# ChuhanZhou/News_Recommendation_Model

Measured on AMD Instinct MI355X. Metric: train impressions/sec, higher is better.
Workload: dtype f32

## Files before the change

### include/nrm_hotpath.h

```cpp
#ifndef NRM_HOTPATH_H
#define NRM_HOTPATH_H

#ifdef __cplusplus
extern "C" {
#endif

#define NRM_ABI_VERSION 7
#define NRM_OK 0
#define NRM_EINVAL (-1)
#define NRM_ELAUNCH (-2)

typedef void* nrm_stream_t;

int nrm_abi_version(void);
const char* nrm_last_error(void);
int nrm_build_flags(void);
const char* nrm_source_digest(void);
const char* nrm_build_info(void);


#define NRM_MMA_F32 0
#define NRM_MMA_BF16 1
#define NRM_MMA_BF16X3 2
long nrm_pwattn_packed_floats(int D);
int nrm_pwattn_pack_wp(const float* fc1_weight, int ld, int D, int mma, float* packed, nrm_stream_t stream);
int nrm_pwattn_fwd(const float* t, const float* h, const float* u, const float* v, const float* packed_wp,
                   const float* w2, const float* b2, float* z, float* s,
                   int B, int T, int H, int D, int mma, nrm_stream_t stream);

#define NRM_DZ_F32 0
#define NRM_DZ_HL4 1
int nrm_pwattn_bwd_dz(float* z_inout, const float* ds, const float* w2, float* dw2, float* db2, float* du, float* dv,
                      int B, int T, int H, int D, int dz_format, nrm_stream_t stream);
int nrm_pwattn_bwd_nsplit(int B, int T, int H, int D, int mma);
int nrm_pwattn_bwd_contract(const float* dz, const float* t, const float* h, const float* wp, int ldwp,
                            float* dt, float* dh, float* ws,
                            int B, int T, int H, int D, int passes, int mma, int dz_format, nrm_stream_t stream);
int nrm_pwattn_bwd_form(int T, int H, int D, int pass, int mma, int dz_format);
int nrm_pwattn_bwd_rw_supported(int D, int mma);
long nrm_pwattn_bwd_rw_packed_floats(int D, int mma);
int nrm_pwattn_bwd_rw_pack(const float* fc1_weight, int ld, int D, int mma, float* packed, nrm_stream_t stream);
int nrm_pwattn_bwd_rw_dtdh(const float* dz_hl4, const float* t, const float* h, const float* packed, float* dt, float* dh,
                           int B, int T, int H, int D, int mma, nrm_stream_t stream);

int nrm_pwattn_bwd_dp_supported(int D, int H);
long nrm_pwattn_bwd_dp_packed_floats(int D, int H);
int nrm_pwattn_bwd_dp_pack(const float* fc1_weight, int ld, int D, int H, float* packed, nrm_stream_t stream);
int nrm_pwattn_bwd_dp_dtdh(const float* dz, const float* t, const float* h, const float* packed, float* dt, float* dh,
                           int B, int T, int H, int D, nrm_stream_t stream);

#define NRM_EPI_BIAS 0
#define NRM_EPI_GELU 1
#define NRM_EPI_DGELU 2
#define NRM_EPI_MUL 3
long nrm_gemm_packed_floats(int nrows, int ncols, int mma);
int nrm_gemm_nt_bf16_supported(int M, int K, int mma);
int nrm_gemm_pack(const float* src, long row_stride, long col_stride, int nrows, int ncols, float* packed,
                  nrm_stream_t stream);
typedef struct {
    const float* src; const float* src2; float sign2;
    long row_stride, col_stride; int nrows, ncols;
    float* packed;
    int mma;
} nrm_pack_desc;
int nrm_gemm_pack_multi(const nrm_pack_desc* descs, int n, nrm_stream_t stream);
int nrm_gemm_nt(const float* x, int ldx, int M, const float* packed, int N, int K, const float* bias,
                float* y, int ldy, float* z, int ldz, const float* m, int ldm, int epilogue, int mma, nrm_stream_t stream);
int nrm_gemm_tn_nsplit(int ncols_i, int ncols_j, int R, int mma);
int nrm_gemm_tn(const float* A, int lda, int ncols_i, const float* B, int ldb, int ncols_j, int R,
                float* ws, int ldws, float* colsum, float* zero_out, long zero_n, int mma, nrm_stream_t stream);

int nrm_slab_reduce(const float* ws, int nsplit, int nj, int ldws, int ni, float* out, long out_istride, long out_jstride,
                    float* out2, long out2_istride, long out2_jstride, float sign2,
                    const float* vec, float* vec_out, nrm_stream_t stream);
typedef struct nrm_slab_desc {
    const float* ws; int nsplit, nj, ldws, ni;
    float* out; long out_istride, out_jstride;
    float* out2; long out2_istride, out2_jstride; float sign2;
    const float* vec; float* vec_out;
} nrm_slab_desc;
int nrm_slab_reduce_multi(const nrm_slab_desc* descs, int n, nrm_stream_t stream);

int nrm_head_fold(const float* w_o1, const float* b_o1, const float* w_m2, const float* b_m2, int P, int Q, int R,
                  float* packed_fwd, float* packed_bwd, float* bias, nrm_stream_t stream);
int nrm_head_fold_bwd(const float* dwp, int ldp, const float* dbp, const float* w_o1, const float* w_m2, const float* b_m2,
                      int P, int Q, int R, float* dw_o1, float* dw_m2, float* db_o1, float* db_m2, nrm_stream_t stream);

int nrm_colreduce(int mode, const float* x, const float* dy, const float* mean, const float* rstd,
                  float* s0, float* s1, int R, int N, int ld, nrm_stream_t stream);
int nrm_bn_finalize(int stage, const float* s, float* out, float* running, int R, int N, float momentum, float eps,
                    nrm_stream_t stream);
// ... 98 lines not shown
```

### news_recommendation_model_amd/csrc/capi.hip

```cpp
#include <stdarg.h>
#include <stdint.h>
#include <stdio.h>
#include <stdlib.h>
#include <vector>

#include "../../include/nrm_hotpath.h"
#include "pwattn.hpp"
#include "gemm.hpp"
#include "head.hpp"
#include "pool_loss.hpp"
#include "frontend.hpp"
#include "scoring.hpp"
#include "compact.hpp"

static thread_local char g_err[512] = "";

static int fail(int code, const char* fmt, ...) {
    va_list ap;
    va_start(ap, fmt);
    vsnprintf(g_err, sizeof(g_err), fmt, ap);
    va_end(ap);
    return code;
}
static int check_hip(hipError_t e, const char* what) {
// ... 201 lines not shown
    if (!fc1_weight || !packed) return fail(NRM_EINVAL, "nrm_pwattn_bwd_dp_pack: null pointer");
    if (D <= 0 || D % 4 || ld < 4 * D) return fail(NRM_EINVAL, "nrm_pwattn_bwd_dp_pack: D=%d ld=%d (need D%%4==0, ld>=4D)", D, ld);
    if (!nrm_pwattn_bwd_dp_supported(D, H)) return fail(NRM_EINVAL, "nrm_pwattn_bwd_dp_pack: D=%d H=%d has no dP-walk backward", D, H);
    return check_hip(nrm::pwattn_bwd_dp_pack_launch(fc1_weight + 3 * (long)D, ld, D, H, packed, (hipStream_t)stream), "bwd_dp_pack");
}

int nrm_pwattn_bwd_dp_dtdh(const float* dz, const float* t, const float* h, const float* packed, float* dt, float* dh,
                           int B, int T, int H, int D, nrm_stream_t stream) {
    if (int rc = check_dims("nrm_pwattn_bwd_dp_dtdh", B, T, H, D)) return rc;
    if (!dz || !t || !h || !packed || !dt || !dh) return fail(NRM_EINVAL, "nrm_pwattn_bwd_dp_dtdh: null pointer");
    if (!nrm_pwattn_bwd_dp_supported(D, H)) return fail(NRM_EINVAL, "nrm_pwattn_bwd_dp_dtdh: D=%d H=%d has no dP-walk backward (D %% 4 == 0, H >= 16)", D, H);
    if ((long)(63 / H + 2) * T * H * D * 4 >= (1L << 31)) return fail(NRM_EINVAL, "nrm_pwattn_bwd_dp_dtdh: the dz blocks of one row block exceed 2^31 bytes");
    if ((long)B * H * D * 4 >= (1L << 31) || (long)B * T * D * 4 >= (1L << 31)) return fail(NRM_EINVAL, "nrm_pwattn_bwd_dp_dtdh: t or h exceeds 2^31 bytes");
    if (B == 0) return NRM_OK;
    nrm::BwdDpParams p = {};
    p.dz = dz; p.t = t; p.h = h; p.wimg = packed; p.dt = dt; p.dh = dh; p.B = B; p.T = T; p.H = H; p.D = D;
    p.w_bytes = (unsigned)(nrm_pwattn_bwd_dp_packed_floats(D, H) * 4);
    p.t_bytes = (unsigned)((long)B * T * D * 4); p.h_bytes = (unsigned)((long)B * H * D * 4);
    return check_hip(nrm::pwattn_bwd_dp_launch(p, (hipStream_t)stream), "bwd_dp_dtdh");
}

int nrm_pwattn_bwd_nsplit(int B, int T, int H, int D, int mma) {
    if (B <= 0 || T <= 0 || H <= 0 || D <= 0) return 0;
    return bwd_bt_plan(B, T, D, mma).nsplit;
}

int nrm_pwattn_bwd_contract(const float* dz, const float* t, const float* h, const float* wp, int ldwp,
                            float* dt, float* dh, float* ws, int B, int T, int H, int D, int passes, int mma,
                            int dz_format, nrm_stream_t stream) {
    if (int rc = check_dims("nrm_pwattn_bwd_contract", B, T, H, D)) return rc;
    if (int rc = check_mma("nrm_pwattn_bwd_contract", mma)) return rc;
    if (passes != 1 && passes != 2 && passes != 3 && passes != 4) return fail(NRM_EINVAL, "nrm_pwattn_bwd_contract: passes=%d", passes);
    if (!bwd_dz_format_ok(passes, mma, dz_format))
        return fail(NRM_EINVAL, "nrm_pwattn_bwd_contract: passes=%d mma=%d with dz_format=%d (only the dW_p-only pass, 4, of the bf16 arithmetics reads NRM_DZ_HL4)", passes, mma, dz_format);
    if (!dz || !t || !h || !wp) return fail(NRM_EINVAL, "nrm_pwattn_bwd_contract: null pointer");
    if (((passes & 1) && (!dt || !ws)) || ((passes & 2) && !dh) || (passes == 4 && !ws)) return fail(NRM_EINVAL, "nrm_pwattn_bwd_contract: null output");
    if (ldwp < D || ldwp % 4) return fail(NRM_EINVAL, "nrm_pwattn_bwd_contract: ldwp=%d", ldwp);
    if (B == 0) return NRM_OK;
    for (int pass : {passes == 4 ? 4 : passes & 1, passes & 2}) {
        if (!pass) continue;
        const BwdPass a = bwd_pass(pass, dz, t, h, wp, ldwp, dt, dh, ws, B, T, H, D, mma, dz_format);
        if (int rc = check_hip(nrm::bwd_e_launch(a.p, a.pl, a.with_dw, mma, (hipStream_t)stream), pass == 2 ? "bwd_e pass 2" : "bwd_e pass 1")) return rc;
    }
    return NRM_OK;
}

int nrm_pwattn_bwd_form(int T, int H, int D, int pass, int mma, int dz_format) {
    if (check_dims("nrm_pwattn_bwd_form", 1, T, H, D) || check_mma("nrm_pwattn_bwd_form", mma)) return -1;
    if ((pass != 1 && pass != 2 && pass != 4) || !bwd_dz_format_ok(pass, mma, dz_format)) return -1;
    const BwdPass a = bwd_pass(pass, nullptr, nullptr, nullptr, nullptr, D, nullptr, nullptr, nullptr, 1, T, H, D, mma, dz_format);
    const nrm::BwdEForm f = nrm::bwd_e_select(a.p, a.pl, a.with_dw, mma, nrm::bwd_e_knobs());
    if (f.family == nrm::BWD_E_REFUSED) return -1;
    return f.family | (f.exact ? 4 : 0) | (a.pl.DT == 5 ? 8 : 0) | (f.with_dw ? 16 : 0) | (f.with_dt ? 32 : 0) | (f.xhl4 ? 64 : 0);
}

static bool al16(const void* p) { return ((uintptr_t)p & 15) == 0; }

long nrm_gemm_packed_floats(int nrows, int ncols, int mma) {
    if (nrows <= 0 || ncols <= 0) return 0;
    if (mma == NRM_MMA_BF16 || mma == NRM_MMA_BF16X3)
        return (long)((nrows + 15) / 16) * ((ncols + 31) / 32) * (mma == NRM_MMA_BF16X3 ? 2 : 1) * 256 + 1024;
    const nrm::GemmNtPlan pl = nrm::gemm_nt_plan(nrows);
    return (long)((ncols + 15) / 16) * pl.rows * 16 + 1024;
}

int nrm_gemm_nt_bf16_supported(int M, int K, int mma) { return nrm::gemm_nt_rx_bm(M, K, mma) ? 1 : 0; }

int nrm_gemm_pack(const float* src, long row_stride, long col_stride, int nrows, int ncols, float* packed,
                  nrm_stream_t stream) {
    if (!src || !packed || nrows <= 0 || ncols <= 0) return fail(NRM_EINVAL, "nrm_gemm_pack: bad argument");
    const nrm::GemmNtPlan pl = nrm::gemm_nt_plan(nrows);
    return check_hip(nrm::pack_rows_launch(src, row_stride, col_stride, nrows, ncols, pl.rows, (ncols + 15) / 16, packed,
                                           (hipStream_t)stream), "pack_rows");
}

int nrm_gemm_pack_multi(const nrm_pack_desc* descs, int n, nrm_stream_t stream) {
    if (n < 0 || (n > 0 && !descs)) return fail(NRM_EINVAL, "nrm_gemm_pack_multi: bad argument");
    for (int lo = 0; lo < n; lo += nrm::PACK_MAX) {
        const int m = n - lo < nrm::PACK_MAX ? n - lo : nrm::PACK_MAX;
        nrm::PackTable tab = {};
        long mx = 0;
        for (int i = 0; i < m; ++i) {
            const nrm_pack_desc& d = descs[lo + i];
            if (!d.src || !d.packed || d.nrows <= 0 || d.ncols <= 0) return fail(NRM_EINVAL, "nrm_gemm_pack_multi: entry %d is malformed", lo + i);
            const nrm::GemmNtPlan pl = nrm::gemm_nt_plan(d.nrows);
            nrm::PackEntry& e = tab.e[i];
            e.src = d.src; e.src2 = d.src2; e.dst = d.packed; e.rs = d.row_stride; e.cs = d.col_stride;
            e.nrows = d.nrows; e.ncols = d.ncols; e.rows = pl.rows; e.kchunks = (d.ncols + 15) / 16; e.sign2 = d.sign2; e.fmt = 0;
            if (d.mma == NRM_MMA_BF16 || d.mma == NRM_MMA_BF16X3) {
                e.fmt = d.mma == NRM_MMA_BF16X3 ? 2 : 1; e.rows = (d.nrows + 15) / 16 * 16; e.kchunks = (d.ncols + 31) / 32;
            } else if (d.mma != NRM_MMA_F32) return fail(NRM_EINVAL, "nrm_gemm_pack_multi: entry %d: mma=%d", lo + i, d.mma);
            const long total = e.fmt ? (long)(e.rows / 16) * e.kchunks * 512 : (long)e.kchunks * e.rows * 16;
            if (total > mx) mx = total;
        }
        if (int rc = check_hip(nrm::pack_rows_multi_launch(tab, m, mx, (hipStream_t)stream), "pack_rows_multi")) return rc;
    }
    return NRM_OK;
}

int nrm_gemm_nt(const float* x, int ldx, int M, const float* packed, int N, int K, const float* bias,
                float* y, int ldy, float* z, int ldz, const float* m, int ldm, int epilogue, int mma, nrm_stream_t stream) {
    if (!x || !packed || !y) return fail(NRM_EINVAL, "nrm_gemm_nt: null pointer");
    if (M < 0 || N <= 0 || K <= 0) return fail(NRM_EINVAL, "nrm_gemm_nt: M=%d N=%d K=%d", M, N, K);
    if (ldx % 4 || ldy % 4 || ldx < K || ldy < N || !al16(x) || !al16(y))
        return fail(NRM_EINVAL, "nrm_gemm_nt: ldx=%d ldy=%d must be multiples of 4 covering K=%d / N=%d, rows 16-B aligned", ldx, ldy, K, N);
    if (epilogue != NRM_EPI_BIAS && (!z || ldz % 4 || ldz < N || !al16(z)))
// ... 501 lines not shown
```

### news_recommendation_model_amd/csrc/pwattn.hpp

```cpp
#pragma once
#include <hip/hip_runtime.h>

namespace nrm {

struct FwdParams {
    const float* t;
    const float* h;
    const float* u;
    const float* v;
    const float* wp;
    const float* w2;
    const float* b2;
    float* z;
    float* s;
    long M;
    int T, H, D;
    int ldt, ldh, ldu, ldv;
    unsigned wp_bytes, t_bytes, h_bytes;
    int rows;
    int kchunks;
    int nchunks;
};
struct RaggedTabs {
    const int* cand_imp;
    const int* cand_off;
    int B, N;
    int max_count;
    const int* hist_off;
    const int* tile_pre;
    const int4* tile_tab;
    int R, Mt, k_max;
};
struct FwdPlan { int NT, MT, nchunks, rows, kchunks; };
FwdPlan pwattn_fwd_plan(int D);
hipError_t pwattn_fwd_launch(const FwdParams& p, const FwdPlan& pl, int mma, hipStream_t st);
hipError_t pwattn_fwd_ragged_launch(const FwdParams& p, const FwdPlan& pl, const RaggedTabs& rg, hipStream_t st);
hipError_t pwattn_fwd_hragged_launch(const FwdParams& p, const FwdPlan& pl, const RaggedTabs& rg, hipStream_t st);
hipError_t pack_wp_launch(const float* w, int ldw, int D, const FwdPlan& pl, int mma, float* packed, hipStream_t st);
struct RwPlan { int nts, nsplit, rows, k32, wimg; };
RwPlan pwattn_rw_plan(int D, int mma);
bool pwattn_fwd_uses_rw(int D, int mma);
hipError_t pwattn_fwd_rw_launch(const FwdParams& p, int mma, hipStream_t st);
hipError_t pwattn_fwd_rw_ragged_launch(const FwdParams& p, const RaggedTabs& rg, hipStream_t st);
hipError_t pwattn_fwd_rw_hragged_launch(const FwdParams& p, const RaggedTabs& rg, hipStream_t st);
hipError_t pack_wp_bf16_launch(const float* w, int ldw, int D, int mma, float* packed, hipStream_t st);

struct BwdEParams {
    const float* X; long xs1, xs2, xrs;
    const float* Y; long ys1, yrs;
    const float* wp; int ldwp;
    const float* srow; int lds_;
    float* out; int ldo;
    float* ws;
    int G, G2, R, D;
    int gps;
    int nkw, ndcol;
    int nsplit;
    int interleave;
    int x_hl4;
    int with_dt;
    int order;
};
struct BwdEPlan { int DT, KT, ndcol, nkw, nsplit, gps; };
BwdEPlan bwd_e_plan(int D, int G, int target_waves, int min_gps = 1, int mma = 0);
enum BwdEFamily { BWD_E_REFUSED = -1, BWD_E_SERIAL = 0, BWD_E_PIPE = 1, BWD_DW_DIRECT = 2, BWD_DW_R32 = 3 };
struct BwdEKnobs { bool pipe, dw_direct, dw_r32; };
BwdEKnobs bwd_e_knobs();
struct BwdEForm {
    int family;
    bool with_dw, with_dt, xhl4; int ks;
    bool exact; int mma;
};
BwdEForm bwd_e_select(const BwdEParams& p, const BwdEPlan& pl, bool with_dw, int mma, const BwdEKnobs& knobs);
hipError_t bwd_e_launch(const BwdEParams& p, const BwdEPlan& pl, bool with_dw, int mma, hipStream_t st);
hipError_t bwd_dz_launch(float* z, const float* ds, const float* w2, float* dw2, float* db2, float* du, float* dv,
                         int B, int T, int H, int D, int dz_format, hipStream_t st);

struct BwdRwParams {
    const float* dz;
    const float* t;
    const float* h;
    const float* wimg;
    float* dt;
    float* dh;
    int B, T, H, D;
    unsigned w_bytes;
    int tsplit;
};
struct BwdRwPlan { int ng, kc, nks, wimg, k32, rows; };
BwdRwPlan pwattn_bwd_rw_plan(int D, int mma);
long pwattn_bwd_rw_packed_floats(int D, int mma);
hipError_t pwattn_bwd_rw_pack_launch(const float* wp, int ldw, int D, int mma, float* packed, hipStream_t st);
hipError_t pwattn_bwd_rw_launch(const BwdRwParams& p, int mma, hipStream_t st);

struct BwdDpParams {
    const float* dz;
    const float* t;
    const float* h;
    const float* wimg;
    float* dt;
    float* dh;
    int B, T, H, D;
    unsigned w_bytes, t_bytes, h_bytes;
    int rows, kchunks, nchunks;
    long steps;
};
struct BwdDpPlan { int NT, nchunks, rows, kchunks; };
BwdDpPlan pwattn_bwd_dp_plan(int D, int H);
long pwattn_bwd_dp_packed_floats(int D, int H);
hipError_t pwattn_bwd_dp_pack_launch(const float* wp, int ldw, int D, int H, float* packed, hipStream_t st);
hipError_t pwattn_bwd_dp_launch(BwdDpParams p, hipStream_t st);

int pwattn_fwd_diag_flags();
int pwattn_fwd_rw_diag_flags();
int pwattn_bwd_rw_diag_flags();
int pwattn_bwd_dp_diag_flags();
int pwattn_bwd_diag_flags();

}
```

### news_recommendation_model_amd/csrc/pwattn_bwd.hip

```cpp
#include <cstdlib>
#include <type_traits>
#ifndef NRM_PRIO
#define NRM_PRIO 0
#endif
#ifndef NRM_PIPE_SGB
#define NRM_PIPE_SGB 1
#endif
#ifndef NRM_EPI_AHEAD
#define NRM_EPI_AHEAD 1
#endif
#ifndef NRM_DIAG_GELU_AT_LOAD
#define NRM_DIAG_GELU_AT_LOAD 0
#endif
#ifndef NRM_DIAG_NOEPI
#define NRM_DIAG_NOEPI 0
#endif
#ifndef NRM_DIAG_NOATOM
#define NRM_DIAG_NOATOM 0
#endif
#ifndef NRM_DIAG_NOLOAD
#define NRM_DIAG_NOLOAD 0
#endif
#include "common.hpp"
#include "pwattn.hpp"
// ... 675 lines not shown
            if (lg >= g_hi) return;
            if (ls == 0) open_group(lg);
            const u32x4 va = __builtin_amdgcn_raw_buffer_load_b128(rx, vx4, ls * xstep, 0);
            const u32x4 vb = __builtin_amdgcn_raw_buffer_load_b128(ry, vy4, ls * ystep, 0);
#pragma unroll
            for (int e = 0; e < 4; ++e) { a[e] = __uint_as_float(va[e]); b[e] = __uint_as_float(vb[e]); }
            if (KT > 4) a[4] = __uint_as_float(__builtin_amdgcn_raw_buffer_load_b32(rx, vx1, ls * xstep, 0));
            if (DT > 4) b[4] = __uint_as_float(__builtin_amdgcn_raw_buffer_load_b32(ry, vy1, ls * ystep, 0));
            if (++ls == nsteps) { ls = 0; lg += g_step; }
        };
        int cs = 0;
        auto consume = [&](const float (&a)[KT], const float (&b)[DT]) {
            if (cs == 0) {
#pragma unroll
                for (int jt = 0; jt < DT; ++jt) sr_cur[jt] = sr_nxt[jt];
            }
            float bs[DT];
#pragma unroll
            for (int jt = 0; jt < DT; ++jt) bs[jt] = b[jt] * sr_cur[jt];
            e_mfma<KT, DT>(dW, a, bs);
            if (++cs == nsteps) cs = 0;
        };
        const int ngroups = (g_hi - g_lo + g_step - 1) / g_step;
        const int total = ngroups * nsteps;
#pragma unroll
        for (int u = 0; u < NSET; ++u) request(a[u], b[u]);
        for (int n = 0; n < total; n += NSET) {
#pragma unroll
            for (int u = 0; u < NSET; ++u)
                if (u == 0 || n + u < total) {
                    consume(a[u], b[u]);
                    request(a[u], b[u]);
                }
        }
    }

    float* wsp = p.ws + (long)split * D * D;
#pragma unroll
    for (int jt = 0; jt < DT; ++jt) {
        const int d = d0 + tn_col<DT>(jt, r16);
        if (!(EXACT || d < D)) continue;
        float* row = wsp + (long)d * D + k0;
#pragma unroll
        for (int e = 0; e < 4; ++e) {
            const int kk = 16 * q + 4 * e;
            if (EXACT || k0 + kk < D)
                *reinterpret_cast<f32x4*>(row + kk) = f32x4{dW[0][jt][e], dW[1][jt][e], dW[2][jt][e], dW[3][jt][e]};
        }
        if (KT > 4 && (EXACT || k0 + 64 + 4 * q < D)) *reinterpret_cast<f32x4*>(row + 64 + 4 * q) = dW[KT - 1][jt];
    }
#endif
}

template <int KT, int DT, bool EXACT>
__global__ __launch_bounds__(256, 2) void bwd_e_pipe_kernel(const BwdEParams p) {
#if defined(__HIP_DEVICE_COMPILE__)
    constexpr int PE = (DT + 1) & ~1;
    constexpr int LDK = KT * 16 + 8;
    __shared__ __attribute__((aligned(16))) float smem[DT * 16 * LDK + 4 * DT * 16];
    float* wpt = smem;
    const int tid = threadIdx.x;
    const int lane = tid & 63;
    const int wave = __builtin_amdgcn_readfirstlane(tid >> 6);
    float* bounce = smem + DT * 16 * LDK + wave * (DT * 16);
    const int r16 = lane & 15, q = lane >> 4;
    const int D = p.D, R = p.R;

    const ETile tl = e_tile<KT, DT, false>(p);
    const int d0 = tl.d0, k0 = tl.k0, sgrp = tl.sgrp;

    for (int idx = tid; idx < KT * 16 * DT * 4; idx += 256) {
        const int kl = idx / (DT * 4), d4 = idx - kl * (DT * 4);
        const int k = k0 + kl, d = d0 + 4 * d4;
        f32x4 w = f32x4{0.f, 0.f, 0.f, 0.f};
        if (k < D && d < D) w = *reinterpret_cast<const f32x4*>(p.wp + (long)k * p.ldwp + d);
#pragma unroll
        for (int e = 0; e < 4; ++e) wpt[tile_pos(4 * d4 + e) * LDK + tile_pos(kl)] = w[e];
    }
    __syncthreads();

    const int split = sgrp * 4 + wave;
    if (split >= p.nsplit) return;
    const EGroups gr = e_groups<false>(p, sgrp, wave);
    const int g_lo = gr.lo, g_hi = gr.hi;
    if (g_lo >= g_hi) return;
    const int nsteps = (R + 3) >> 2;

    const unsigned vx4 = (EXACT || k0 + 4 * r16 < D) ? (unsigned)((long)q * p.xrs + k0 + 4 * r16) * 4u : BUF_OOB;
    const unsigned vx1 = (EXACT || k0 + 64 + r16 < D) ? (unsigned)((long)q * p.xrs + k0 + 64 + r16) * 4u : BUF_OOB;
    const unsigned vy4 = (EXACT || d0 + 4 * r16 < D) ? (unsigned)((long)q * p.yrs + d0 + 4 * r16) * 4u : BUF_OOB;
    const unsigned vy1 = (EXACT || d0 + 64 + r16 < D) ? (unsigned)((long)q * p.yrs + d0 + 64 + r16) * 4u : BUF_OOB;
    const unsigned xbytes = (unsigned)(((long)(R - 1) * p.xrs + D) * 4);
    const unsigned ybytes = (unsigned)(((long)(R - 1) * p.yrs + D) * 4);
    const int xstep = (int)(p.xrs * 16), ystep = (int)(p.yrs * 16);

    float a0[KT], b0[DT], a1[KT], b1[DT];
    __amdgpu_buffer_rsrc_t rx, ry, rxn, ryn;
    auto open_group = [&](int gg, __amdgpu_buffer_rsrc_t& ox, __amdgpu_buffer_rsrc_t& oy) {
        const EOperands o = e_open(p, gg, xbytes, ybytes);
        ox = o.x; oy = o.y;
    };
    bool diag_first = true;
    auto load_step = [&](__amdgpu_buffer_rsrc_t dx, __amdgpu_buffer_rsrc_t dy, float (&a)[KT], float (&b)[DT], int s) {
        if (NRM_DIAG_NOLOAD == 1 && !(diag_first && s < 2)) return;
        const u32x4 va = __builtin_amdgcn_raw_buffer_load_b128(dx, vx4, s * xstep, 0);
        const u32x4 vb = __builtin_amdgcn_raw_buffer_load_b128(dy, vy4, s * ystep, 0);
// ... 173 lines not shown
                f32x4 c = f32x4{0.f, 0.f, 0.f, 0.f};
                if (MMA == 2) {
                    c = __builtin_amdgcn_mfma_f32_16x16x32_bf16(al, ybf[jt], c, 0, 0, 0);
                    c = __builtin_amdgcn_mfma_f32_16x16x32_bf16(af, ybl[jt], c, 0, 0, 0);
                }
                E[it][jt] = __builtin_amdgcn_mfma_f32_16x16x32_bf16(af, ybf[jt], c, 0, 0, 0);
            }
        }
#pragma unroll
        for (int jt = 0; jt < DT; ++jt)
#pragma unroll
            for (int it = 0; it < KT; ++it) dW[it][jt] += E[it][jt] * sr[jt];
    }

    float* wsp = p.ws + (long)split * D * D;
#pragma unroll
    for (int jt = 0; jt < DT; ++jt) {
        const int d = d0 + 4 * r16 + jt;
        if (!(EXACT || d < D)) continue;
        float* row = wsp + (long)d * D + k0;
#pragma unroll
        for (int e = 0; e < 4; ++e) {
            const int kk = 16 * q + 4 * e;
            if (EXACT || k0 + kk < D)
                *reinterpret_cast<f32x4*>(row + kk) = f32x4{dW[0][jt][e], dW[1][jt][e], dW[2][jt][e], dW[3][jt][e]};
        }
    }
#endif
}

BwdEPlan bwd_e_plan(int D, int G, int target_waves, int min_gps, int mma) {
    const int n16 = (D + 15) / 16;
    const int c5 = (n16 + 4) / 5 * 5, c4 = (n16 + 3) / 4 * 4;
    BwdEPlan pl;
    if (c5 < c4) { pl.DT = 5; pl.KT = 5; } else { pl.DT = 4; pl.KT = 4; }
    if (mma != 0) { pl.DT = 4; pl.KT = 4; }
    pl.ndcol = (n16 + pl.DT - 1) / pl.DT;
    pl.nkw = (n16 + pl.KT - 1) / pl.KT;
    const int tiles = pl.ndcol * pl.nkw;
    int ns = target_waves / tiles / 4 * 4;
    if (min_gps > 1 && ns > G / min_gps) {
        const int one_round = 2048 / tiles / 4 * 4;
        if (one_round >= 4 && one_round < ns) ns = one_round;
    }
    if (ns < 4) ns = 4;
    if (ns > G) ns = G > 0 ? G : 1;
    pl.gps = (G + ns - 1) / ns;
    pl.nsplit = pl.gps > 0 ? (G + pl.gps - 1) / pl.gps : 1;
    return pl;
}

BwdEKnobs bwd_e_knobs() {
    auto on = [](const char* name) { const char* e = getenv(name); return !(e && e[0] == '0'); };
    return {on("NRM_BH_PIPE"), on("NRM_DW_DIRECT"), on("NRM_DW_R32")};
}

BwdEForm bwd_e_select(const BwdEParams& p, const BwdEPlan& pl, bool with_dw, int mma, const BwdEKnobs& knobs) {
    const int KT = pl.KT, DT = pl.DT;
    const BwdEForm refused = {BWD_E_REFUSED, false, false, false, 0, false, mma};
    BwdEForm f = {BWD_E_SERIAL, with_dw, true, false, DT, p.D % (16 * KT) == 0 && p.D % (16 * DT) == 0, mma};
    if (KT != 4) {
        if (mma != 0) return refused;
    } else if (mma == 1 || mma == 2) {
        if (!p.with_dt && !p.x_hl4) {
            if (!with_dw) return refused;
            f.with_dt = false;
        } else if (!p.with_dt || p.x_hl4) {
            if (!with_dw || p.with_dt || !p.x_hl4) return refused;
            f.with_dt = false; f.xhl4 = true;
            if (knobs.dw_r32 && p.R <= 32) f.family = BWD_DW_R32;
        }
        return f;
    }
    f.mma = 0;
    if (with_dw && !p.with_dt) {
        if (p.x_hl4) return refused;
        f.with_dt = false;
        if (knobs.dw_direct && (p.R + 3) / 4 >= DW_SETS) f.family = BWD_DW_DIRECT;
    } else if (!with_dw && knobs.pipe && (p.R + 3) / 4 >= ((DT + 1) & ~1) + 2) {
        f.family = BWD_E_PIPE;
    }
    return f;
}

template <class F>
static void with_tile_exact_mma(int tile, bool exact, int mma, F&& f) {
    auto go = [&](auto t, auto m) { return exact ? f(t, std::true_type{}, m) : f(t, std::false_type{}, m); };
    using T4 = std::integral_constant<int, 4>;
    if (tile == 5) return go(std::integral_constant<int, 5>{}, std::integral_constant<int, 0>{});
    if (mma == 1) return go(T4{}, std::integral_constant<int, 1>{});
    if (mma == 2) return go(T4{}, std::integral_constant<int, 2>{});
    return go(T4{}, std::integral_constant<int, 0>{});
}

int pwattn_bwd_diag_flags() {
    return (NRM_EPI_AHEAD != 1 ? 8 : 0) | (NRM_DIAG_GELU_AT_LOAD ? 16 : 0) | (NRM_DIAG_NOEPI ? 32 : 0) | (NRM_DIAG_NOATOM ? 64 : 0) |
           (NRM_DIAG_NOLOAD ? 128 : 0) | (NRM_PIPE_SGB != 1 ? 256 : 0);
}

hipError_t bwd_e_launch(const BwdEParams& params, const BwdEPlan& pl, bool with_dw, int mma, hipStream_t st) {
    if (params.G <= 0) return hipSuccess;
    const BwdEForm f = bwd_e_select(params, pl, with_dw, mma, bwd_e_knobs());
    BwdEParams p = params;
    p.nkw = pl.nkw; p.ndcol = pl.ndcol; p.gps = pl.gps; p.nsplit = pl.nsplit;
    const dim3 grid(pl.nkw * pl.ndcol, (pl.nsplit + 3) / 4), block(256);
    hipError_t rc = hipErrorInvalidValue;
    if (f.family != BWD_E_REFUSED) with_tile_exact_mma(pl.DT, f.exact, f.mma, [&](auto tile, auto exact, auto arith) {
        constexpr int KT = decltype(tile)::value, DT = KT, MMA = decltype(arith)::value;
        constexpr bool EXACT = decltype(exact)::value;
        constexpr std::true_type Y{}; constexpr std::false_type N{};
        auto serial = [&](auto dw, auto dt, auto xhl4) {
            hipLaunchKernelGGL((bwd_e_kernel<KT, DT, DT, decltype(dw)::value, EXACT, MMA, decltype(dt)::value, decltype(xhl4)::value>), grid, block, 0, st, p);
        };
        if (f.family == BWD_E_SERIAL) {
            if (!f.with_dw) serial(N, Y, N);
            else if (f.with_dt) serial(Y, Y, N);
            else if (!f.xhl4) serial(Y, N, N);
            else if constexpr (MMA != 0) serial(Y, N, Y);
            else return;
        } else if constexpr (MMA == 0) {
            if (f.family == BWD_E_PIPE) hipLaunchKernelGGL((bwd_e_pipe_kernel<KT, DT, EXACT>), grid, block, 0, st, p);
            else if (f.family == BWD_DW_DIRECT) hipLaunchKernelGGL((bwd_dw_direct_kernel<KT, DT, EXACT>), grid, block, 0, st, p);
            else return;
        } else {
            if (f.family == BWD_DW_R32) hipLaunchKernelGGL((bwd_dw_r32_kernel<EXACT, MMA>), grid, block, 0, st, p);
            else return;
        }
        rc = hipGetLastError();
    });
    return rc;
}

}
```

### news_recommendation_model_amd/native.py

```python
from __future__ import annotations

import ctypes
import os
import threading

_HERE = os.path.dirname(os.path.abspath(__file__))
LIB_PATH = os.environ.get("NRM_HOTPATH_LIB") or os.path.join(_HERE, "libnrm_hotpath.so")
ABI_VERSION = 7

_c_fp = ctypes.c_void_p
_c_i, _c_l = ctypes.c_int, ctypes.c_long

SIGNATURES = {
    "nrm_abi_version": (_c_i, []),
    "nrm_last_error": (ctypes.c_char_p, []),
    "nrm_build_flags": (_c_i, []),
    "nrm_source_digest": (ctypes.c_char_p, []),
    "nrm_build_info": (ctypes.c_char_p, []),
    "nrm_pwattn_packed_floats": (_c_l, [_c_i]),
    "nrm_pwattn_pack_wp": (_c_i, [_c_fp, _c_i, _c_i, _c_i, _c_fp, _c_fp]),
    "nrm_pwattn_fwd": (_c_i, [_c_fp] * 9 + [_c_i] * 5 + [_c_fp]),
    "nrm_pwattn_bwd_dz": (_c_i, [_c_fp] * 7 + [_c_i] * 5 + [_c_fp]),
    "nrm_pwattn_bwd_rw_supported": (_c_i, [_c_i, _c_i]),
    "nrm_pwattn_bwd_rw_packed_floats": (_c_l, [_c_i, _c_i]),
    "nrm_pwattn_bwd_rw_pack": (_c_i, [_c_fp, _c_i, _c_i, _c_i, _c_fp, _c_fp]),
    "nrm_pwattn_bwd_rw_dtdh": (_c_i, [_c_fp] * 6 + [_c_i] * 5 + [_c_fp]),
    "nrm_pwattn_bwd_dp_supported": (_c_i, [_c_i, _c_i]),
    "nrm_pwattn_bwd_dp_packed_floats": (_c_l, [_c_i, _c_i]),
    "nrm_pwattn_bwd_dp_pack": (_c_i, [_c_fp, _c_i, _c_i, _c_i, _c_fp, _c_fp]),
    "nrm_pwattn_bwd_dp_dtdh": (_c_i, [_c_fp] * 6 + [_c_i] * 4 + [_c_fp]),
    "nrm_pwattn_bwd_nsplit": (_c_i, [_c_i] * 5),
    "nrm_pwattn_bwd_contract": (_c_i, [_c_fp] * 4 + [_c_i] + [_c_fp] * 3 + [_c_i] * 7 + [_c_fp]),
    "nrm_pwattn_bwd_form": (_c_i, [_c_i] * 6),
    "nrm_gemm_packed_floats": (_c_l, [_c_i, _c_i, _c_i]),
    "nrm_gemm_nt_bf16_supported": (_c_i, [_c_i, _c_i, _c_i]),
    "nrm_gemm_pack": (_c_i, [_c_fp, _c_l, _c_l, _c_i, _c_i, _c_fp, _c_fp]),
    "nrm_gemm_nt": (_c_i, [_c_fp, _c_i, _c_i, _c_fp, _c_i, _c_i, _c_fp, _c_fp, _c_i, _c_fp, _c_i, _c_fp, _c_i, _c_i, _c_i, _c_fp]),
    "nrm_slab_reduce": (_c_i, [_c_fp, _c_i, _c_i, _c_i, _c_i, _c_fp, _c_l, _c_l, _c_fp, _c_l, _c_l, ctypes.c_float,
                               _c_fp, _c_fp, _c_fp]),
    "nrm_bn_finalize": (_c_i, [_c_i, _c_fp, _c_fp, _c_fp, _c_i, _c_i, ctypes.c_float, ctypes.c_float, _c_fp]),
    "nrm_mul_bwd": (_c_i, [_c_fp, _c_i, _c_fp, _c_i, _c_fp, _c_i, _c_fp, _c_fp, _c_i, _c_i, _c_i, _c_fp]),
    "nrm_gemm_tn_nsplit": (_c_i, [_c_i, _c_i, _c_i, _c_i]),
    "nrm_gemm_tn": (_c_i, [_c_fp, _c_i, _c_i, _c_fp, _c_i, _c_i, _c_i, _c_fp, _c_i, _c_fp, _c_fp, _c_l, _c_i, _c_fp]),
    "nrm_gemm_pack_multi": (_c_i, [_c_fp, _c_i, _c_fp]),
    "nrm_slab_reduce_multi": (_c_i, [_c_fp, _c_i, _c_fp]),
    "nrm_head_fold": (_c_i, [_c_fp] * 4 + [_c_i] * 3 + [_c_fp] * 4),
    "nrm_head_fold_bwd": (_c_i, [_c_fp, _c_i, _c_fp, _c_fp, _c_fp, _c_fp, _c_i, _c_i, _c_i] + [_c_fp] * 5),
    "nrm_colreduce": (_c_i, [_c_i] + [_c_fp] * 6 + [_c_i] * 3 + [_c_fp]),
    "nrm_bn_apply": (_c_i, [_c_fp] * 6 + [_c_i] * 3 + [_c_fp]),
    "nrm_bn_backward": (_c_i, [_c_fp] * 9 + [_c_i] * 4 + [_c_fp]),
    "nrm_concat_cols": (_c_i, [_c_fp, _c_fp, _c_fp, _c_i, _c_fp, _c_i, _c_l, _c_fp]),
    "nrm_pool_bmm": (_c_i, [_c_fp, _c_l, _c_l, _c_l, _c_fp, _c_i, _c_fp] + [_c_i] * 5 + [_c_fp]),
    "nrm_pool_rowdot": (_c_i, [_c_fp, _c_i, _c_fp, _c_fp] + [_c_i] * 4 + [_c_fp, _c_i, _c_fp]),
    "nrm_small_linear_relu_fwd": (_c_i, [_c_fp, _c_i, _c_fp, _c_fp, _c_fp, _c_l, _c_i, _c_i, _c_i, _c_fp]),
    "nrm_small_linear_relu_bwd": (_c_i, [_c_fp, _c_i, _c_fp, _c_fp, _c_fp, _c_i, _c_l, _c_i, _c_i, _c_fp, _c_fp]),
    "nrm_loss_fwd_bwd": (_c_i, [_c_fp, _c_i, _c_fp, _c_i, _c_fp, _c_fp, _c_l, ctypes.c_float, _c_i, _c_i, _c_fp, _c_fp, _c_i, _c_fp, _c_fp, _c_fp]),
    "nrm_adam_step": (_c_i, [_c_fp] * 4 + [_c_l] + [ctypes.c_float] * 5 + [_c_i, _c_i, _c_fp]),
    "nrm_adam_step_dev": (_c_i, [_c_fp] * 4 + [_c_l] + [ctypes.c_float] * 5 + [_c_fp, _c_i, _c_fp]),
    "nrm_gather_flat": (_c_i, [_c_fp, _c_fp, _c_fp, _c_i, _c_fp, _c_l, _c_fp]),
    "nrm_row_auc": (_c_i, [_c_fp] * 3 + [_c_i, _c_i] + [_c_fp] * 3),
    "nrm_ensemble_rank_max_candidates": (_c_i, []),
    "nrm_ensemble_rank": (_c_i, [_c_fp] * 3 + [_c_i, _c_fp, _c_fp, _c_i, _c_i] + [_c_fp] * 5),
    "nrm_compact_gather": (_c_i, [_c_fp, _c_i, _c_i, _c_fp, _c_i, _c_i, _c_fp, _c_fp, _c_i, _c_i, _c_i, _c_i, _c_fp, _c_fp, _c_fp, _c_fp]),
    "nrm_pwattn_fwd_ragged": (_c_i, [_c_fp] * 10 + [_c_i] * 6 + [_c_fp]),
    "nrm_pool_bmm_ragged": (_c_i, [_c_fp] * 4 + [_c_i] * 5 + [_c_fp]),
    "nrm_history_len": (_c_i, [_c_fp, _c_i, _c_i, _c_i, _c_i, _c_fp, _c_fp]),
    "nrm_history_gather": (_c_i, [_c_fp, _c_i, _c_i, _c_fp, _c_i, _c_i, _c_i, _c_i, _c_fp, _c_fp]),
    "nrm_history_tiles": (_c_i, [_c_fp] * 4 + [_c_i] * 4 + [_c_fp, _c_fp]),
    "nrm_pwattn_fwd_hragged": (_c_i, [_c_fp] * 13 + [_c_i] * 8 + [_c_fp]),
    "nrm_pool_bmm_hragged": (_c_i, [_c_fp] * 7 + [_c_i] * 7 + [_c_fp]),
    "nrm_history_gather_groups": (_c_i, [_c_fp, _c_i, _c_i] + [_c_fp] * 4 + [_c_i] * 4 + [_c_fp, _c_fp]),
    "nrm_pool_bmm_wlast": (_c_i, [_c_fp, _c_l, _c_l, _c_l, _c_fp, _c_i, _c_fp] + [_c_i] * 5 + [ctypes.c_float, _c_i, _c_fp]),
    "nrm_pool_rowdot_wlast": (_c_i, [_c_fp, _c_i, _c_fp, _c_fp] + [_c_i] * 4 + [_c_fp, _c_i, ctypes.c_float, _c_fp]),
    "nrm_ensemble_rank_ragged": (_c_i, [_c_fp, _c_fp, _c_i, _c_fp, _c_fp, _c_i, _c_fp, _c_i, _c_i] + [_c_fp] * 5),
    "nrm_frontend_fwd": (_c_i, [_c_fp, _c_i, _c_i, _c_i, _c_i, _c_i, _c_i,  _c_fp, _c_i, _c_i,  _c_fp, _c_fp, _c_i,
                                 _c_fp, _c_i, _c_i,  _c_fp, _c_fp, _c_fp, _c_fp,  _c_i, _c_i, _c_i, _c_i, _c_i,
                                 _c_fp, _c_i, _c_fp, _c_i, _c_fp, _c_fp]),
    "nrm_frontend_tables_ws_floats": (_c_l, [_c_l] + [_c_i] * 9),
    "nrm_frontend_bwd_tables": (_c_i, [_c_fp, _c_i, _c_i, _c_i, _c_fp, _c_i] * 2 + [_c_i] * 3 + [_c_fp, _c_fp] + [_c_i] * 9
                                + [_c_fp] * 8 + [_c_fp]),
    "nrm_frontend_cat_ws_ints": (_c_l, [_c_i, _c_l, _c_i]),
    "nrm_frontend_cat_grad": (_c_i, [_c_fp, _c_i, _c_i, _c_fp, _c_i] * 2 + [_c_i] * 5 + [_c_fp, _c_fp, _c_fp]),
    "nrm_frontend_bwd": (_c_i, [_c_fp, _c_i, _c_i, _c_i, _c_i, _c_i, _c_i,  _c_fp, _c_i, _c_fp, _c_fp]
                         + [_c_i] * 10 + [_c_fp] * 8 + [_c_fp]),
}

# ... 84 lines not shown
```

Before: 35880.

## Add packed-group dW kernel for pairwise-attention backward when R is not a multiple of four

Adds a bwd_dw_pack_kernel that packs 2 or 4 consecutive groups into one 4-row MFMA K-step when the per-group row count R is not divisible by 4. This avoids the padded, partially wasted MFMA steps and buffer loads the direct dW kernel spends on ragged row tails. Selection is gated by stride contiguity, the group count per split and 32-bit offset checks. It falls back to the existing direct kernel otherwise, and adds an env knob plus a query API.

After: 36580 (median of 6 runs). +2.0%, better.

```diff
diff --git a/include/nrm_hotpath.h b/include/nrm_hotpath.h
--- a/include/nrm_hotpath.h
+++ b/include/nrm_hotpath.h
@@ -37,6 +37,7 @@
                             float* dt, float* dh, float* ws,
                             int B, int T, int H, int D, int passes, int mma, int dz_format, nrm_stream_t stream);
 int nrm_pwattn_bwd_form(int T, int H, int D, int pass, int mma, int dz_format);
+int nrm_pwattn_bwd_dw_pack(int B, int T, int H, int D, int mma);
 int nrm_pwattn_bwd_rw_supported(int D, int mma);
 long nrm_pwattn_bwd_rw_packed_floats(int D, int mma);
 int nrm_pwattn_bwd_rw_pack(const float* fc1_weight, int ld, int D, int mma, float* packed, nrm_stream_t stream);
diff --git a/news_recommendation_model_amd/csrc/capi.hip b/news_recommendation_model_amd/csrc/capi.hip
--- a/news_recommendation_model_amd/csrc/capi.hip
+++ b/news_recommendation_model_amd/csrc/capi.hip
@@ -277,6 +277,13 @@
     const nrm::BwdEForm f = nrm::bwd_e_select(a.p, a.pl, a.with_dw, mma, nrm::bwd_e_knobs());
     if (f.family == nrm::BWD_E_REFUSED) return -1;
     return f.family | (f.exact ? 4 : 0) | (a.pl.DT == 5 ? 8 : 0) | (f.with_dw ? 16 : 0) | (f.with_dt ? 32 : 0) | (f.xhl4 ? 64 : 0);
+}
+
+int nrm_pwattn_bwd_dw_pack(int B, int T, int H, int D, int mma) {
+    if (B <= 0 || check_dims("nrm_pwattn_bwd_dw_pack", B, T, H, D) || check_mma("nrm_pwattn_bwd_dw_pack", mma)) return -1;
+    const BwdPass a = bwd_pass(4, nullptr, nullptr, nullptr, nullptr, D, nullptr, nullptr, nullptr, B, T, H, D, mma, NRM_DZ_F32);
+    const nrm::BwdEForm f = nrm::bwd_e_select(a.p, a.pl, a.with_dw, mma, nrm::bwd_e_knobs());
+    return f.family == nrm::BWD_DW_DIRECT ? f.pack : 1;
 }
 
 static bool al16(const void* p) { return ((uintptr_t)p & 15) == 0; }
diff --git a/news_recommendation_model_amd/csrc/pwattn.hpp b/news_recommendation_model_amd/csrc/pwattn.hpp
--- a/news_recommendation_model_amd/csrc/pwattn.hpp
+++ b/news_recommendation_model_amd/csrc/pwattn.hpp
@@ -64,12 +64,13 @@
 struct BwdEPlan { int DT, KT, ndcol, nkw, nsplit, gps; };
 BwdEPlan bwd_e_plan(int D, int G, int target_waves, int min_gps = 1, int mma = 0);
 enum BwdEFamily { BWD_E_REFUSED = -1, BWD_E_SERIAL = 0, BWD_E_PIPE = 1, BWD_DW_DIRECT = 2, BWD_DW_R32 = 3 };
-struct BwdEKnobs { bool pipe, dw_direct, dw_r32; };
+struct BwdEKnobs { bool pipe, dw_direct, dw_r32, dw_pack; };
 BwdEKnobs bwd_e_knobs();
 struct BwdEForm {
     int family;
     bool with_dw, with_dt, xhl4; int ks;
     bool exact; int mma;
+    int pack = 1;
 };
 BwdEForm bwd_e_select(const BwdEParams& p, const BwdEPlan& pl, bool with_dw, int mma, const BwdEKnobs& knobs);
 hipError_t bwd_e_launch(const BwdEParams& p, const BwdEPlan& pl, bool with_dw, int mma, hipStream_t st);
diff --git a/news_recommendation_model_amd/csrc/pwattn_bwd.hip b/news_recommendation_model_amd/csrc/pwattn_bwd.hip
--- a/news_recommendation_model_amd/csrc/pwattn_bwd.hip
+++ b/news_recommendation_model_amd/csrc/pwattn_bwd.hip
@@ -751,6 +751,138 @@
 #endif
 }
 
+#if defined(__HIP_DEVICE_COMPILE__)
+template <int KT, int DT, bool EXACT, int PP, int NSET>
+__device__ __forceinline__ void dw_pack_walk(const BwdEParams& p, f32x4 (&dW)[KT][DT], int g_lo, int g_hi, int d0, int k0, int lane) {
+    const int D = p.D, R = p.R;
+    const int steps = PP == 1 ? (R + 3) >> 2 : (PP * R) >> 2;
+    const int rstep = PP == 1 ? 4 : 1;
+    auto group_of = [](int q) { return PP == 1 ? 0 : PP == 2 ? q >> 1 : q; };
+    auto row_of = [&](int q) { return PP == 1 ? q : PP == 2 ? (q & 1) * steps : 0; };
+    unsigned vx4, vx1;
+    {
+        const int r16 = lane & 15, q = lane >> 4;
+        const long xrow = (long)(group_of(q) * R + row_of(q)) * p.xrs;
+        vx4 = (EXACT || k0 + 4 * r16 < D) ? (unsigned)(xrow + k0 + 4 * r16) * 4u : BUF_OOB;
+        vx1 = (EXACT || k0 + 64 + r16 < D) ? (unsigned)(xrow + k0 + 64 + r16) * 4u : BUF_OOB;
+    }
+    const unsigned xbytes = (unsigned)(((long)(PP * R - 1) * p.xrs + D) * 4);
+    const unsigned ybytes = (unsigned)(((long)(R - 1) * p.yrs + D) * 4);
+    const unsigned sbytes = (unsigned)(((long)(PP - 1) * p.lds_ + D) * 4);
+    const unsigned yimp = (unsigned)(p.ys1 * 4);
+    const int xstep = (int)(p.xrs * 4) * rstep, ystep = (int)(p.yrs * 4) * rstep;
+    if (g_lo >= g_hi) return;
+
+    float a[NSET][KT], b[NSET][DT];
+    float sr_cur[DT], sr_nxt[DT];
+    __amdgpu_buffer_rsrc_t rx, ry;
+    unsigned vy4 = BUF_OOB, vy1 = BUF_OOB;
+    int lg = g_lo, ls = 0;
+    auto open_unit = [&](int gg) {
+        int l = lane;
+        asm volatile("" : "+v"(l));
+        const int r16 = l & 15, q = l >> 4, j = group_of(q);
+        const int g1 = gg / p.G2, g2 = gg - g1 * p.G2;
+        rx = buffer_rsrc(p.X + (long)g1 * p.xs1 + (long)g2 * p.xs2, xbytes);
+        unsigned mine = 0, last = 0;
+        if (PP > 1) {
+            int rl = g2 + j, ru = g2 + PP - 1;
+#pragma unroll
+            for (int i = 1; i < PP; ++i) {
+                if (rl >= p.G2) { rl -= p.G2; ++mine; }
+                if (ru >= p.G2) { ru -= p.G2; ++last; }
+            }
+            last = __builtin_amdgcn_readfirstlane(last);
+        }
+        const unsigned yrow = mine * yimp + (unsigned)(row_of(q) * (int)p.yrs) * 4u, srw = (unsigned)(j * p.lds_) * 4u;
+        const bool ok4 = EXACT || d0 + 4 * r16 < D, ok1 = EXACT || d0 + 64 + r16 < D;
+        vy4 = ok4 ? yrow + (unsigned)(d0 + 4 * r16) * 4u : BUF_OOB;
+        vy1 = ok1 ? yrow + (unsigned)(d0 + 64 + r16) * 4u : BUF_OOB;
+        ry = buffer_rsrc(p.Y + (long)g1 * p.ys1, last * yimp + ybytes);
+        const __amdgpu_buffer_rsrc_t rs = buffer_rsrc(p.srow + (long)gg * p.lds_, sbytes);
+        const u32x4 s4 = __builtin_amdgcn_raw_buffer_load_b128(rs, ok4 ? srw + (unsigned)(d0 + 4 * r16) * 4u : BUF_OOB, 0, 0);
+#pragma unroll
+        for (int e = 0; e < 4; ++e) sr_nxt[e] = __uint_as_float(s4[e]);
+        if (DT > 4) sr_nxt[4] = __uint_as_float(__builtin_amdgcn_raw_buffer_load_b32(rs, ok1 ? srw + (unsigned)(d0 + 64 + r16) * 4u : BUF_OOB, 0, 0));
+    };
+    auto request = [&](float (&a)[KT], float (&b)[DT]) {
+        if (lg >= g_hi) return;
+        if (ls == 0) open_unit(lg);
+        const u32x4 va = __builtin_amdgcn_raw_buffer_load_b128(rx, vx4, ls * xstep, 0);
+        const u32x4 vb = __builtin_amdgcn_raw_buffer_load_b128(ry, vy4, ls * ystep, 0);
+#pragma unroll
+        for (int e = 0; e < 4; ++e) { a[e] = __uint_as_float(va[e]); b[e] = __uint_as_float(vb[e]); }
+        if (KT > 4) a[4] = __uint_as_float(__builtin_amdgcn_raw_buffer_load_b32(rx, vx1, ls * xstep, 0));
+        if (DT > 4) b[4] = __uint_as_float(__builtin_amdgcn_raw_buffer_load_b32(ry, vy1, ls * ystep, 0));
+        if (++ls == steps) { ls = 0; lg += PP; }
+    };
+    int cs = 0;
+    auto consume = [&](const float (&a)[KT], const float (&b)[DT]) {
+        if (cs == 0) {
+#pragma unroll
+            for (int jt = 0; jt < DT; ++jt) sr_cur[jt] = sr_nxt[jt];
+        }
+        float bs[DT];
+#pragma unroll
+        for (int jt = 0; jt < DT; ++jt) bs[jt] = b[jt] * sr_cur[jt];
+        e_mfma<KT, DT>(dW, a, bs);
+        if (++cs == steps) cs = 0;
+    };
+    const int total = (g_hi - g_lo) / PP * steps;
+#pragma unroll
+    for (int u = 0; u < NSET; ++u) request(a[u], b[u]);
+    for (int n = 0; n < total; n += NSET) {
+#pragma unroll
+        for (int u = 0; u < NSET; ++u)
+            if (u == 0 || n + u < total) {
+                consume(a[u], b[u]);
+                request(a[u], b[u]);
+            }
+    }
+}
+#endif
+
+template <int KT, int DT, bool EXACT, int P, int NSET = DW_SETS>
+__global__ __launch_bounds__(256, DW_WPE) void bwd_dw_pack_kernel(const BwdEParams p) {
+#if defined(__HIP_DEVICE_COMPILE__)
+    static_assert(P == 2 || P == 4, "P = 4 / gcd(R, 4) groups per super-group; P = 1 is bwd_dw_direct_kernel");
+    const int tid = threadIdx.x;
+    const int lane = tid & 63;
+    const int wave = __builtin_amdgcn_readfirstlane(tid >> 6);
+    const int r16 = lane & 15, q = lane >> 4;
+    const int D = p.D;
+    const ETile tl = e_tile<KT, DT, true>(p);
+    const int d0 = tl.d0, k0 = tl.k0, sgrp = tl.sgrp;
+    const int split = sgrp * 4 + wave;
+    if (split >= p.nsplit) return;
+    const EGroups gr = e_groups<false>(p, sgrp, wave);
+    const int g_mid = gr.lo + (gr.hi > gr.lo ? (gr.hi - gr.lo) / P * P : 0);
+
+    f32x4 dW[KT][DT];
+#pragma unroll
+    for (int it = 0; it < KT; ++it)
+#pragma unroll
+        for (int jt = 0; jt < DT; ++jt) dW[it][jt] = f32x4{0.f, 0.f, 0.f, 0.f};
+    dw_pack_walk<KT, DT, EXACT, P, NSET>(p, dW, gr.lo, g_mid, d0, k0, lane);
+    dw_pack_walk<KT, DT, EXACT, 1, NSET>(p, dW, g_mid, gr.hi, d0, k0, lane);
+
+    float* wsp = p.ws + (long)split * D * D;
+#pragma unroll
+    for (int jt = 0; jt < DT; ++jt) {
+        const int d = d0 + tn_col<DT>(jt, r16);
+        if (!(EXACT || d < D)) continue;
+        float* row = wsp + (long)d * D + k0;
+#pragma unroll
+        for (int e = 0; e < 4; ++e) {
+            const int kk = 16 * q + 4 * e;
+            if (EXACT || k0 + kk < D)
+                *reinterpret_cast<f32x4*>(row + kk) = f32x4{dW[0][jt][e], dW[1][jt][e], dW[2][jt][e], dW[3][jt][e]};
+        }
+        if (KT > 4 && (EXACT || k0 + 64 + 4 * q < D)) *reinterpret_cast<f32x4*>(row + 64 + 4 * q) = dW[KT - 1][jt];
+    }
+#endif
+}
+
 template <int KT, int DT, bool EXACT>
 __global__ __launch_bounds__(256, 2) void bwd_e_pipe_kernel(const BwdEParams p) {
 #if defined(__HIP_DEVICE_COMPILE__)
@@ -1030,7 +1162,15 @@
 
 BwdEKnobs bwd_e_knobs() {
     auto on = [](const char* name) { const char* e = getenv(name); return !(e && e[0] == '0'); };
-    return {on("NRM_BH_PIPE"), on("NRM_DW_DIRECT"), on("NRM_DW_R32")};
+    return {on("NRM_BH_PIPE"), on("NRM_DW_DIRECT"), on("NRM_DW_R32"), on("NRM_DW_PACK")};
+}
+
+static int bwd_dw_pack(const BwdEParams& p, const BwdEPlan& pl) {
+    const int P = p.R % 4 == 0 ? 1 : p.R % 2 == 0 ? 2 : 4;
+    if (P == 1 || p.interleave || pl.gps < P || P * p.R / 4 < DW_SETS) return 1;
+    if (p.xs2 != (long)p.R * p.xrs || p.xs1 != (long)p.G2 * p.xs2 || p.xrs < p.D || p.ys1 < (long)(p.R - 1) * p.yrs + p.D || p.lds_ < p.D) return 1;
+    if ((long)P * p.R * p.xrs * 4 >= (1L << 31) || (long)P * p.ys1 * 4 >= (1L << 31) || (long)P * p.lds_ * 4 >= (1L << 31)) return 1;
+    return P;
 }
 
 BwdEForm bwd_e_select(const BwdEParams& p, const BwdEPlan& pl, bool with_dw, int mma, const BwdEKnobs& knobs) {
@@ -1055,6 +1195,7 @@
         if (p.x_hl4) return refused;
         f.with_dt = false;
         if (knobs.dw_direct && (p.R + 3) / 4 >= DW_SETS) f.family = BWD_DW_DIRECT;
+        if (f.family == BWD_DW_DIRECT && knobs.dw_pack) f.pack = bwd_dw_pack(p, pl);
     } else if (!with_dw && knobs.pipe && (p.R + 3) / 4 >= ((DT + 1) & ~1) + 2) {
         f.family = BWD_E_PIPE;
     }
@@ -1098,7 +1239,10 @@
             else return;
         } else if constexpr (MMA == 0) {
             if (f.family == BWD_E_PIPE) hipLaunchKernelGGL((bwd_e_pipe_kernel<KT, DT, EXACT>), grid, block, 0, st, p);
-            else if (f.family == BWD_DW_DIRECT) hipLaunchKernelGGL((bwd_dw_direct_kernel<KT, DT, EXACT>), grid, block, 0, st, p);
+            else if (f.family != BWD_DW_DIRECT) return;
+            else if (f.pack == 1) hipLaunchKernelGGL((bwd_dw_direct_kernel<KT, DT, EXACT>), grid, block, 0, st, p);
+            else if (f.pack == 2) hipLaunchKernelGGL((bwd_dw_pack_kernel<KT, DT, EXACT, 2>), grid, block, 0, st, p);
+            else if (f.pack == 4) hipLaunchKernelGGL((bwd_dw_pack_kernel<KT, DT, EXACT, 4>), grid, block, 0, st, p);
             else return;
         } else {
             if (f.family == BWD_DW_R32) hipLaunchKernelGGL((bwd_dw_r32_kernel<EXACT, MMA>), grid, block, 0, st, p);
diff --git a/news_recommendation_model_amd/native.py b/news_recommendation_model_amd/native.py
--- a/news_recommendation_model_amd/native.py
+++ b/news_recommendation_model_amd/native.py
@@ -32,6 +32,7 @@
     "nrm_pwattn_bwd_nsplit": (_c_i, [_c_i] * 5),
     "nrm_pwattn_bwd_contract": (_c_i, [_c_fp] * 4 + [_c_i] + [_c_fp] * 3 + [_c_i] * 7 + [_c_fp]),
     "nrm_pwattn_bwd_form": (_c_i, [_c_i] * 6),
+    "nrm_pwattn_bwd_dw_pack": (_c_i, [_c_i] * 5),
     "nrm_gemm_packed_floats": (_c_l, [_c_i, _c_i, _c_i]),
     "nrm_gemm_nt_bf16_supported": (_c_i, [_c_i, _c_i, _c_i]),
     "nrm_gemm_pack": (_c_i, [_c_fp, _c_l, _c_l, _c_i, _c_i, _c_fp, _c_fp]),
```
